# AshishKumar4/FlaxDiff

Hardware: AMD Instinct MI355X
Metric: train images/sec/node (64x64 uncond EDM UNet, bs=256) (higher is better)
Workload: dtype bf16; 1 GPU; model=unet_64px_[64,128,256,512]_res2_heads4, global_batch=256, resolution=64, parallelism=dp1, schedule=EDM + KarrasPredictionTransform(sigma_data=0.5)

## Files before the change

flaxdiff_amd/ops/hip/conv2d_halo_v2.hip:

```cpp
#include <torch/extension.h>
#include <ATen/hip/HIPContext.h>
#include "common.h"
#include "host_util.h"

typedef __bf16 bf16v8h __attribute__((ext_vector_type(8)));

#define HV2_NTH 256
#define HV2_BK 64

union HBF8 { bf16v8h v; ushort u[8]; uint4 q; };

__device__ __forceinline__ void hv2_glds16(const ushort* src, ushort* dst) {
    __builtin_amdgcn_global_load_lds(
        (const __attribute__((address_space(1))) void*)src,
        (__attribute__((address_space(3))) void*)dst, 16, 0, 0);
}

template <bool TRANSPOSED, int BMT, int BNT, int W, bool UP = false>
__global__ __launch_bounds__(HV2_NTH, 2)
void conv2d_halo_v2_kernel(
        const ushort* __restrict__ X,
        const ushort* __restrict__ Wt,
        const float* __restrict__ bias,
        const ushort* __restrict__ addp,
        const ushort* __restrict__ baddp,
        ushort* __restrict__ Y,
        const int Bn, const int R,
        const int Cin, const int Cout,
        const long M) {
    constexpr int RPT = BMT / W;
    constexpr int NSLOT = RPT + 2;
    constexpr int NROW_H = NSLOT * (W + 2);
    constexpr int ZR = NROW_H;
    constexpr int WB0 = NROW_H + 3;
    constexpr int NW = BNT / 32;
    constexpr int NHC = (NSLOT * W / 8 + 3) / 4;
    constexpr int WMW = BMT / 64;

    extern __shared__ __attribute__((aligned(16))) ushort hlds[];
    const int tid = threadIdx.x;
    const int lane = tid & 63;
    const int wid = tid >> 6;
    const int wn = wid / WMW;
    const int wm = wid % WMW;
    const int half = lane >> 5;
    const int l31 = lane & 31;

    const long m_base = (long)blockIdx.x * BMT;
    const int n_base = blockIdx.y * BNT;
    const long grow0 = m_base / W;
    const long BH = (long)Bn * R;
    const int ksl = Cin / HV2_BK;

    for (int i = tid; i < 3 * 64; i += HV2_NTH)
        hlds[ZR * 64 + i] = 0;
    for (int i = tid; i < NSLOT * 2 * 64; i += HV2_NTH) {
        const int sl = i >> 7;
        const int e = (i >> 6) & 1;
        hlds[(sl * (W + 2) + (e ? (W + 1) : 0)) * 64 + (i & 63)] = 0;
    }
    __syncthreads();

    int brow[2][3];
    #pragma unroll
    for (int fm = 0; fm < 2; ++fm) {
        const long m = m_base + wm * 64 + fm * 32 + l31;
        const long mc = m < M ? m : M - 1;
        const int ow = (int)(mc % W);
        const long grow = mc / W;
        const int orow = (int)(grow % R);
        #pragma unroll
        for (int dr = -1; dr <= 1; ++dr) {
            if (m >= M || orow + dr < 0 || orow + dr >= R) {
                brow[fm][dr + 1] = ZR + 1;
            } else {
                const int slot = (int)(grow + dr - grow0) + 1;
                brow[fm][dr + 1] = slot * (W + 2) + ow + 1;
            }
        }
    }

    auto issue_halo = [&](int ci0) {
        #pragma unroll
        for (int i = 0; i < NHC; ++i) {
            int q = wid + i * 4;
            const int qmax = NSLOT * W / 8 - 1;
            q = q > qmax ? qmax : q;
            const int slot = q / (W / 8);
            const int c = q % (W / 8);
            long g = grow0 + slot - 1;
            g = g < 0 ? 0 : (g >= BH ? BH - 1 : g);
            const int pos0 = c * 8;
            const int rowbase = slot * (W + 2) + 1 + pos0;
            const int pix = pos0 + (lane >> 3);
            const int key = (rowbase + (lane >> 3)) & 7;
            const ushort* s;
            if (UP) {
                const int b = (int)(g / R);
                const int r = (int)(g - (long)b * R);
                const long gs = (long)b * (R >> 1) + (r >> 1);
                s = X + (gs * (W >> 1) + (pix >> 1)) * (long)Cin + ci0
                  + (((lane & 7) ^ key) << 3);
            } else {
                s = X + (g * W + pix) * (long)Cin + ci0
                  + (((lane & 7) ^ key) << 3);
            }
            hv2_glds16(s, hlds + rowbase * 64);
        }
    };
    auto issue_w = [&](int flat, int last) {
        const int f = flat > last ? last : flat;
        const int tap = f % 9;
        const int ci0 = (f / 9) * HV2_BK;
        const ushort* wslab = Wt + (long)tap * Cout * Cin;
        const int buf = (WB0 + (flat % 3) * BNT) * 64;
        #pragma unroll
        for (int i = 0; i < NW; ++i) {
            const int row0 = (wid + i * 4) * 8;
            const int r8 = lane >> 3;
            const int key = ((row0 + r8) & 7);
            const ushort* s = wslab + (long)(n_base + row0 + r8) * Cin + ci0
                            + (((lane & 7) ^ key) << 3);
            hv2_glds16(s, hlds + buf + row0 * 64);
        }
    };

    f32x16 acc[2][2] = {};
    const int nflat = 9 * ksl;

    issue_halo(0);
    issue_w(0, nflat - 1);
    issue_w(1, nflat - 1);

    for (int flat = 0; flat < nflat; ++flat) {
        const int tap = flat % 9;
        const int sci = flat / 9;
        if (tap == 0 && sci > 0) {
            asm volatile("s_waitcnt vmcnt(0)" ::: "memory");
        } else {
            asm volatile("s_waitcnt vmcnt(%0)" :: "i"(NW) : "memory");
        }
        __builtin_amdgcn_s_barrier();
        issue_w(flat + 2, nflat - 1);

        const int r = tap / 3, s = tap % 3;
        const int dr = TRANSPOSED ? (1 - r) : (r - 1);
        const int ds = TRANSPOSED ? (1 - s) : (s - 1);
        const int wbuf = (WB0 + (flat % 3) * BNT) * 64;
        const int ar0 = wn * 64 + l31;
        const int ar1 = ar0 + 32;
        const int br0 = brow[0][dr + 1] + ds;
        const int br1 = brow[1][dr + 1] + ds;
        #pragma unroll
        for (int kk = 0; kk < HV2_BK / 16; ++kk) {
            const int k0 = kk * 16 + half * 8;
            const int ch = k0 >> 3;
            bf16v8h a0 = reinterpret_cast<const HBF8*>(
                hlds + wbuf + ar0 * 64 + ((ch ^ (ar0 & 7)) << 3))->v;
            bf16v8h a1 = reinterpret_cast<const HBF8*>(
                hlds + wbuf + ar1 * 64 + ((ch ^ (ar1 & 7)) << 3))->v;
            bf16v8h b0 = reinterpret_cast<const HBF8*>(
                hlds + br0 * 64 + ((ch ^ (br0 & 7)) << 3))->v;
            bf16v8h b1 = reinterpret_cast<const HBF8*>(
                hlds + br1 * 64 + ((ch ^ (br1 & 7)) << 3))->v;
            acc[0][0] = __builtin_amdgcn_mfma_f32_32x32x16_bf16(a0, b0, acc[0][0], 0, 0, 0);
            acc[0][1] = __builtin_amdgcn_mfma_f32_32x32x16_bf16(a0, b1, acc[0][1], 0, 0, 0);
            acc[1][0] = __builtin_amdgcn_mfma_f32_32x32x16_bf16(a1, b0, acc[1][0], 0, 0, 0);
            acc[1][1] = __builtin_amdgcn_mfma_f32_32x32x16_bf16(a1, b1, acc[1][1], 0, 0, 0);
        }
        if (tap == 8 && sci + 1 < ksl) {
            __builtin_amdgcn_s_barrier();
            issue_halo((sci + 1) * HV2_BK);
        }
    }
    asm volatile("s_waitcnt vmcnt(0)" ::: "memory");

    #pragma unroll
    for (int fm = 0; fm < 2; ++fm) {
        const long m = m_base + wm * 64 + fm * 32 + l31;
        if (m >= M) continue;
        ushort* yrow = Y + m * Cout;
        const ushort* brow = baddp ? baddp + (m / (long)(R * W)) * Cout : nullptr;
        #pragma unroll
        for (int fn = 0; fn < 2; ++fn) {
            #pragma unroll
            for (int q = 0; q < 4; ++q) {
                const int n0 = n_base + wn * 64 + fn * 32 + q * 8 + half * 4;
                if (n0 >= Cout) continue;
                float v0 = acc[fn][fm][q * 4 + 0];
                float v1 = acc[fn][fm][q * 4 + 1];
                float v2 = acc[fn][fm][q * 4 + 2];
                float v3 = acc[fn][fm][q * 4 + 3];
                if (bias) {
                    v0 += bias[n0];
                    v1 += (n0 + 1 < Cout) ? bias[n0 + 1] : 0.f;
                    v2 += (n0 + 2 < Cout) ? bias[n0 + 2] : 0.f;
                    v3 += (n0 + 3 < Cout) ? bias[n0 + 3] : 0.f;
                }
                if (addp && n0 + 4 <= Cout) {
                    const ushort4 av =
                        *reinterpret_cast<const ushort4*>(addp + m * Cout + n0);
                    v0 += bf2f(av.x); v1 += bf2f(av.y);
                    v2 += bf2f(av.z); v3 += bf2f(av.w);
                } else if (addp) {
                    for (int j = 0; j < 4 && n0 + j < Cout; ++j) {
                        const float a = bf2f(addp[m * Cout + n0 + j]);
                        if (j == 0) v0 += a; else if (j == 1) v1 += a;
                        else if (j == 2) v2 += a; else v3 += a;
                    }
                }
                if (brow && n0 + 4 <= Cout) {
                    const ushort4 bv = *reinterpret_cast<const ushort4*>(brow + n0);
                    v0 += bf2f(bv.x); v1 += bf2f(bv.y);
                    v2 += bf2f(bv.z); v3 += bf2f(bv.w);
                } else if (brow) {
                    for (int j = 0; j < 4 && n0 + j < Cout; ++j) {
                        const float bv = bf2f(brow[n0 + j]);
                        if (j == 0) v0 += bv; else if (j == 1) v1 += bv;
                        else if (j == 2) v2 += bv; else v3 += bv;
                    }
                }
                if (n0 + 4 <= Cout) {
                    ushort4 pk;
                    pk.x = f2bf(v0); pk.y = f2bf(v1);
                    pk.z = f2bf(v2); pk.w = f2bf(v3);
                    *reinterpret_cast<ushort4*>(yrow + n0) = pk;
                } else {
                    const float vs[4] = {v0, v1, v2, v3};
                    for (int j = 0; j < 4 && n0 + j < Cout; ++j)
                        yrow[n0 + j] = f2bf(vs[j]);
                }
            }
        }
    }
}

template <int BMT, int BNT, int W>
static size_t hv2_smem() {
    constexpr int NROW = (BMT / W + 2) * (W + 2) + 3 + 3 * BNT;
    return (size_t)NROW * 64 * sizeof(ushort);
}

bool conv2d_halo_v2_launch(const void* x, const void* wt, const float* bias,
                           const ushort* addp, const ushort* baddp,
                           void* y, bool transposed,
                           int B, int R, int W, int Cin, int Cout, long M,
                           hipStream_t stream, bool upsample) {
    FD_FLUSH_STALE();
    if (Cin % 64 || Cout % 64) return false;
    if (W != 8 && W != 16 && W != 32 && W != 64) return false;
    int bmt = (Cout <= 64) ? 256 : 128;
    static const bool w64_256tile = std::getenv("FD_HALO_W64_128TILE") == nullptr;
    if (bmt == 128 && W == 64) {
        if (!w64_256tile) {
            if (Cin / HV2_BK < 2) return false;
        } else {
            bmt = 256;
        }
    }
    const int bnt = 128 * 128 / bmt;
    if (bmt % W) return false;
    if (M % W) return false;

    if (upsample && ((R & 1) || (W & 1))) return false;

    dim3 grid((unsigned)((M + bmt - 1) / bmt), (unsigned)((Cout + bnt - 1) / bnt));
    const int mode = upsample ? 2 : (transposed ? 1 : 0);
    #define HV2_KEY(MODE_, BMT_, W_) (((MODE_) << 16) | ((BMT_) << 7) | (W_))
    #define HV2_CASE(MODE_, BMT_, W_)                                          \
        case HV2_KEY(MODE_, BMT_, W_):                                         \
            fd_launch_lds<conv2d_halo_v2_kernel<(MODE_ == 1), BMT_,            \
                                                128 * 128 / BMT_, W_,          \
                                                (MODE_ == 2)>>(                \
                grid, dim3(HV2_NTH), hv2_smem<BMT_, 128 * 128 / BMT_, W_>(),   \
                stream, (const ushort*)x, (const ushort*)wt, bias, addp,       \
                baddp, (ushort*)y, B, R, Cin, Cout, M);                        \
            break;
    #define HV2_TILE(MODE_, BMT_)                                              \
        HV2_CASE(MODE_, BMT_, 8) HV2_CASE(MODE_, BMT_, 16)                     \
        HV2_CASE(MODE_, BMT_, 32) HV2_CASE(MODE_, BMT_, 64)
    switch (HV2_KEY(mode, bmt, W)) {
        HV2_TILE(0, 128) HV2_TILE(0, 256)
        HV2_TILE(1, 128) HV2_TILE(1, 256)
        HV2_TILE(2, 128) HV2_TILE(2, 256)
        default: return false;
    }
    #undef HV2_TILE
    #undef HV2_CASE
    #undef HV2_KEY
    FD_CHECK_LAUNCH();
    return true;
}
```

Before: 5761 images/s.

## Vectorize halo conv epilogue and overlap its loads with the final tap

```diff
diff --git a/flaxdiff_amd/ops/hip/conv2d_halo_v2.hip b/flaxdiff_amd/ops/hip/conv2d_halo_v2.hip
--- a/flaxdiff_amd/ops/hip/conv2d_halo_v2.hip
+++ b/flaxdiff_amd/ops/hip/conv2d_halo_v2.hip
@@ -15,6 +15,111 @@
         (const __attribute__((address_space(1))) void*)src,
         (__attribute__((address_space(3))) void*)dst, 16, 0, 0);
 }
+
+struct HaloEpilogue {
+    float4 bs[2][2][2];
+    uint4 av[2][2][2], bv[2][2][2];
+
+    __device__ __forceinline__ void load_bias(const float* __restrict__ bias,
+                                              const int nl) {
+        #pragma unroll
+        for (int fn = 0; fn < 2; ++fn) {
+            #pragma unroll
+            for (int p = 0; p < 2; ++p) {
+                const float4* b = reinterpret_cast<const float4*>(
+                    bias + nl + fn * 32 + p * 16);
+                bs[fn][p][0] = b[0];
+                bs[fn][p][1] = b[1];
+            }
+        }
+    }
+
+    __device__ __forceinline__ void load_adds(const ushort* __restrict__ addp,
+                                              const ushort* __restrict__ baddp,
+                                              const long m0, const int nl,
+                                              const long RW, const int Cout,
+                                              const long M) {
+        #pragma unroll
+        for (int fm = 0; fm < 2; ++fm) {
+            const long m = m0 + fm * 32;
+            const long mc = m < M ? m : M - 1;
+            if (addp) {
+                const ushort* a = addp + mc * Cout + nl;
+                #pragma unroll
+                for (int fn = 0; fn < 2; ++fn) {
+                    #pragma unroll
+                    for (int p = 0; p < 2; ++p)
+                        av[fm][fn][p] = *reinterpret_cast<const uint4*>(
+                            a + fn * 32 + p * 16);
+                }
+            }
+            if (baddp) {
+                const ushort* b = baddp
+                    + (long)((unsigned)mc / (unsigned)RW) * Cout + nl;
+                #pragma unroll
+                for (int fn = 0; fn < 2; ++fn) {
+                    #pragma unroll
+                    for (int p = 0; p < 2; ++p)
+                        bv[fm][fn][p] = *reinterpret_cast<const uint4*>(
+                            b + fn * 32 + p * 16);
+                }
+            }
+        }
+    }
+
+    static __device__ __forceinline__ void add_bf8(float (&v)[8], const uint4 u) {
+        const uint w[4] = {u.x, u.y, u.z, u.w};
+        #pragma unroll
+        for (int i = 0; i < 4; ++i) {
+            v[2 * i] += __uint_as_float(w[i] << 16);
+            v[2 * i + 1] += __uint_as_float(w[i] & 0xffff0000u);
+        }
+    }
+
+    __device__ __forceinline__ void finish(const f32x16 (&acc)[2][2],
+                                           const bool has_bias,
+                                           const bool has_add,
+                                           const bool has_badd,
+                                           ushort* __restrict__ Y,
+                                           const long m0, const int nl,
+                                           const int Cout, const long M) const {
+        #pragma unroll
+        for (int fm = 0; fm < 2; ++fm) {
+            const long m = m0 + fm * 32;
+            ushort* yrow = Y + m * Cout + nl;
+            #pragma unroll
+            for (int fn = 0; fn < 2; ++fn) {
+                #pragma unroll
+                for (int p = 0; p < 2; ++p) {
+                    float v[8];
+                    #pragma unroll
+                    for (int j = 0; j < 4; ++j) {
+                        const auto r = __builtin_amdgcn_permlane32_swap(
+                            __float_as_uint(acc[fn][fm][(2 * p) * 4 + j]),
+                            __float_as_uint(acc[fn][fm][(2 * p + 1) * 4 + j]),
+                            false, false);
+                        v[j] = __uint_as_float(r[0]);
+                        v[4 + j] = __uint_as_float(r[1]);
+                    }
+                    if (has_bias) {
+                        const float4 b0 = bs[fn][p][0], b1 = bs[fn][p][1];
+                        v[0] += b0.x; v[1] += b0.y; v[2] += b0.z; v[3] += b0.w;
+                        v[4] += b1.x; v[5] += b1.y; v[6] += b1.z; v[7] += b1.w;
+                    }
+                    if (has_add) add_bf8(v, av[fm][fn][p]);
+                    if (has_badd) add_bf8(v, bv[fm][fn][p]);
+                    uint4 pk;
+                    pk.x = f2bf(v[0]) | ((uint)f2bf(v[1]) << 16);
+                    pk.y = f2bf(v[2]) | ((uint)f2bf(v[3]) << 16);
+                    pk.z = f2bf(v[4]) | ((uint)f2bf(v[5]) << 16);
+                    pk.w = f2bf(v[6]) | ((uint)f2bf(v[7]) << 16);
+                    if (m < M)
+                        *reinterpret_cast<uint4*>(yrow + fn * 32 + p * 16) = pk;
+                }
+            }
+        }
+    }
+};
 
 template <bool TRANSPOSED, int BMT, int BNT, int W, bool UP = false>
 __global__ __launch_bounds__(HV2_NTH, 2)
@@ -52,33 +157,12 @@
     const long BH = (long)Bn * R;
     const int ksl = Cin / HV2_BK;
 
-    for (int i = tid; i < 3 * 64; i += HV2_NTH)
-        hlds[ZR * 64 + i] = 0;
-    for (int i = tid; i < NSLOT * 2 * 64; i += HV2_NTH) {
-        const int sl = i >> 7;
-        const int e = (i >> 6) & 1;
-        hlds[(sl * (W + 2) + (e ? (W + 1) : 0)) * 64 + (i & 63)] = 0;
-    }
-    __syncthreads();
-
-    int brow[2][3];
-    #pragma unroll
-    for (int fm = 0; fm < 2; ++fm) {
-        const long m = m_base + wm * 64 + fm * 32 + l31;
-        const long mc = m < M ? m : M - 1;
-        const int ow = (int)(mc % W);
-        const long grow = mc / W;
-        const int orow = (int)(grow % R);
-        #pragma unroll
-        for (int dr = -1; dr <= 1; ++dr) {
-            if (m >= M || orow + dr < 0 || orow + dr >= R) {
-                brow[fm][dr + 1] = ZR + 1;
-            } else {
-                const int slot = (int)(grow + dr - grow0) + 1;
-                brow[fm][dr + 1] = slot * (W + 2) + ow + 1;
-            }
-        }
-    }
+    const int n_wave = n_base + wn * 64;
+    const bool wave_live = n_wave < Cout;
+    const int nl = n_wave + half * 8;
+    const long m0 = m_base + wm * 64 + l31;
+    HaloEpilogue epi;
+    if (bias && wave_live) epi.load_bias(bias, nl);
 
     auto issue_halo = [&](int ci0) {
         #pragma unroll
@@ -108,10 +192,9 @@
             hv2_glds16(s, hlds + rowbase * 64);
         }
     };
-    auto issue_w = [&](int flat, int last) {
-        const int f = flat > last ? last : flat;
-        const int tap = f % 9;
-        const int ci0 = (f / 9) * HV2_BK;
+    auto issue_w = [&](int flat) {
+        const int tap = flat % 9;
+        const int ci0 = (flat / 9) * HV2_BK;
         const ushort* wslab = Wt + (long)tap * Cout * Cin;
         const int buf = (WB0 + (flat % 3) * BNT) * 64;
         #pragma unroll
@@ -119,7 +202,9 @@
             const int row0 = (wid + i * 4) * 8;
             const int r8 = lane >> 3;
             const int key = ((row0 + r8) & 7);
-            const ushort* s = wslab + (long)(n_base + row0 + r8) * Cin + ci0
+            int co = n_base + row0 + r8;
+            co = co < Cout ? co : Cout - 1;
+            const ushort* s = wslab + (long)co * Cin + ci0
                             + (((lane & 7) ^ key) << 3);
             hv2_glds16(s, hlds + buf + row0 * 64);
         }
@@ -129,19 +214,51 @@
     const int nflat = 9 * ksl;
 
     issue_halo(0);
-    issue_w(0, nflat - 1);
-    issue_w(1, nflat - 1);
-
-    for (int flat = 0; flat < nflat; ++flat) {
+    issue_w(0);
+    issue_w(1);
+
+    for (int i = tid; i < 3 * 64; i += HV2_NTH)
+        hlds[ZR * 64 + i] = 0;
+    for (int i = tid; i < NSLOT * 2 * 64; i += HV2_NTH) {
+        const int sl = i >> 7;
+        const int e = (i >> 6) & 1;
+        hlds[(sl * (W + 2) + (e ? (W + 1) : 0)) * 64 + (i & 63)] = 0;
+    }
+
+    int brow[2][3];
+    #pragma unroll
+    for (int fm = 0; fm < 2; ++fm) {
+        const long m = m0 + fm * 32;
+        const unsigned mc = (unsigned)(m < M ? m : M - 1);
+        const int ow = (int)(mc % W);
+        const unsigned grow = mc / W;
+        const int orow = (int)(grow % (unsigned)R);
+        #pragma unroll
+        for (int dr = -1; dr <= 1; ++dr) {
+            if (m >= M || orow + dr < 0 || orow + dr >= R) {
+                brow[fm][dr + 1] = ZR + 1;
+            } else {
+                const int slot = (int)(grow - (unsigned)grow0) + dr + 1;
+                brow[fm][dr + 1] = slot * (W + 2) + ow + 1;
+            }
+        }
+    }
+
+    auto tap_step = [&](const int flat, const bool last) {
         const int tap = flat % 9;
         const int sci = flat / 9;
-        if (tap == 0 && sci > 0) {
-            asm volatile("s_waitcnt vmcnt(0)" ::: "memory");
+        if (last || (tap == 0 && sci > 0)) {
+            asm volatile("s_waitcnt vmcnt(0) lgkmcnt(0)" ::: "memory");
         } else {
-            asm volatile("s_waitcnt vmcnt(%0)" :: "i"(NW) : "memory");
+            asm volatile("s_waitcnt vmcnt(%0) lgkmcnt(0)" :: "i"(NW) : "memory");
         }
         __builtin_amdgcn_s_barrier();
-        issue_w(flat + 2, nflat - 1);
+        if (last) {
+            if (wave_live)
+                epi.load_adds(addp, baddp, m0, nl, (long)R * W, Cout, M);
+        } else if (flat + 2 < nflat) {
+            issue_w(flat + 2);
+        }
 
         const int r = tap / 3, s = tap % 3;
         const int dr = TRANSPOSED ? (1 - r) : (r - 1);
@@ -168,71 +285,18 @@
             acc[1][0] = __builtin_amdgcn_mfma_f32_32x32x16_bf16(a1, b0, acc[1][0], 0, 0, 0);
             acc[1][1] = __builtin_amdgcn_mfma_f32_32x32x16_bf16(a1, b1, acc[1][1], 0, 0, 0);
         }
-        if (tap == 8 && sci + 1 < ksl) {
+        if (!last && tap == 8) {
             __builtin_amdgcn_s_barrier();
             issue_halo((sci + 1) * HV2_BK);
         }
-    }
-    asm volatile("s_waitcnt vmcnt(0)" ::: "memory");
-
-    #pragma unroll
-    for (int fm = 0; fm < 2; ++fm) {
-        const long m = m_base + wm * 64 + fm * 32 + l31;
-        if (m >= M) continue;
-        ushort* yrow = Y + m * Cout;
-        const ushort* brow = baddp ? baddp + (m / (long)(R * W)) * Cout : nullptr;
-        #pragma unroll
-        for (int fn = 0; fn < 2; ++fn) {
-            #pragma unroll
-            for (int q = 0; q < 4; ++q) {
-                const int n0 = n_base + wn * 64 + fn * 32 + q * 8 + half * 4;
-                if (n0 >= Cout) continue;
-                float v0 = acc[fn][fm][q * 4 + 0];
-                float v1 = acc[fn][fm][q * 4 + 1];
-                float v2 = acc[fn][fm][q * 4 + 2];
-                float v3 = acc[fn][fm][q * 4 + 3];
-                if (bias) {
-                    v0 += bias[n0];
-                    v1 += (n0 + 1 < Cout) ? bias[n0 + 1] : 0.f;
-                    v2 += (n0 + 2 < Cout) ? bias[n0 + 2] : 0.f;
-                    v3 += (n0 + 3 < Cout) ? bias[n0 + 3] : 0.f;
-                }
-                if (addp && n0 + 4 <= Cout) {
-                    const ushort4 av =
-                        *reinterpret_cast<const ushort4*>(addp + m * Cout + n0);
-                    v0 += bf2f(av.x); v1 += bf2f(av.y);
-                    v2 += bf2f(av.z); v3 += bf2f(av.w);
-                } else if (addp) {
-                    for (int j = 0; j < 4 && n0 + j < Cout; ++j) {
-                        const float a = bf2f(addp[m * Cout + n0 + j]);
-                        if (j == 0) v0 += a; else if (j == 1) v1 += a;
-                        else if (j == 2) v2 += a; else v3 += a;
-                    }
-                }
-                if (brow && n0 + 4 <= Cout) {
-                    const ushort4 bv = *reinterpret_cast<const ushort4*>(brow + n0);
-                    v0 += bf2f(bv.x); v1 += bf2f(bv.y);
-                    v2 += bf2f(bv.z); v3 += bf2f(bv.w);
-                } else if (brow) {
-                    for (int j = 0; j < 4 && n0 + j < Cout; ++j) {
-                        const float bv = bf2f(brow[n0 + j]);
-                        if (j == 0) v0 += bv; else if (j == 1) v1 += bv;
-                        else if (j == 2) v2 += bv; else v3 += bv;
-                    }
-                }
-                if (n0 + 4 <= Cout) {
-                    ushort4 pk;
-                    pk.x = f2bf(v0); pk.y = f2bf(v1);
-                    pk.z = f2bf(v2); pk.w = f2bf(v3);
-                    *reinterpret_cast<ushort4*>(yrow + n0) = pk;
-                } else {
-                    const float vs[4] = {v0, v1, v2, v3};
-                    for (int j = 0; j < 4 && n0 + j < Cout; ++j)
-                        yrow[n0 + j] = f2bf(vs[j]);
-                }
-            }
-        }
-    }
+    };
+    for (int flat = 0; flat < nflat - 1; ++flat)
+        tap_step(flat, false);
+    tap_step(nflat - 1, true);
+
+    if (wave_live)
+        epi.finish(acc, bias != nullptr, addp != nullptr, baddp != nullptr,
+                   Y, m0, nl, Cout, M);
 }
 
 template <int BMT, int BNT, int W>
@@ -248,6 +312,7 @@
                            hipStream_t stream, bool upsample) {
     FD_FLUSH_STALE();
     if (Cin % 64 || Cout % 64) return false;
+    if (M >= (1L << 31)) return false;
     if (W != 8 && W != 16 && W != 32 && W != 64) return false;
     int bmt = (Cout <= 64) ? 256 : 128;
     static const bool w64_256tile = std::getenv("FD_HALO_W64_128TILE") == nullptr;
```

Result: faster. 6003 images/s, median of 6 (+4.2%).
